# princeton-computational-imaging/Neural-Volume-Super-Resolution

Hardware: AMD Instinct MI355X
Metric: rendered rays/sec (64+128 samples) at 800x800 Lego-like view (higher is better)
Workload: dtype f32 as 2 f16 limbs (3 MFMA products, f32 acc); 1 GPU; Blender-'lego'-like 800x800 view, 64 coarse + 128 fine samples, tri-plane decoder (3x800^2x48 + 32^2x48 planes, 4+4x128 MLP), 1 view per GPU per step; partition=view

## Files before the change

### neural-volume-super-resolution_amd/csrc/render3.hip

```cpp
#include "pair_core.h"

#include "colour_order.h"
#include "occupancy.h"
#include "nvsr_internal.h"

namespace nvsr {

template <int LZ>
__device__ __forceinline__ void render_pass3_body(const SceneDev& sc, const float* __restrict__ packed, long N, int S,
                                                  const float* __restrict__ rays, const float* __restrict__ z, int lindisp,
                                                  const float* __restrict__ noise, int white,
                                                  float* __restrict__ rgb, float* __restrict__ disp,
                                                  float* __restrict__ acc, float* __restrict__ weights,
                                                  float* __restrict__ depth, float* __restrict__ raw_out, unsigned* __restrict__ flag,
                                                  float* __restrict__ live_z = nullptr, float* __restrict__ live_w = nullptr,
                                                  int* __restrict__ live_n = nullptr, const int* __restrict__ group_slot = nullptr,
                                                  const int* __restrict__ pts = nullptr, const int* __restrict__ pt_steps = nullptr, float* views = nullptr,
                                                  const int* __restrict__ kept = nullptr, const int* __restrict__ kept_n = nullptr) {
    constexpr int LIMBS = LZ & 7;
    constexpr bool ZCOMP = (LZ & 8) != 0;
    constexpr int PHASE = (LZ >> 4) & 7;
    constexpr bool FUSED = PHASE == 0, KEPT = PHASE == 4, DENSITY = PHASE == 1 || KEPT, POINTS = PHASE == 3, COLOUR = PHASE == 2 || POINTS;
    constexpr bool F16 = limb_f16(LIMBS);
    using L = Lds3<LIMBS>;
    constexpr int NP = limb_products(LIMBS);
    constexpr int NSF = 3 * 4 * NP, NSH = 4 * 4 * NP;
    __shared__ __attribute__((aligned(16))) unsigned lds[L::TOTAL];
    NVSR_RACE_PROBE_DELAY(lds);
    Ring3<LIMBS> rs{__builtin_amdgcn_make_buffer_rsrc(const_cast<float*>(packed + limb_region(LIMBS)), 0, KB_TOTAL * kb_words(region_limbs(LIMBS)) * 4, 0x00020000),
                    lds, 0, __builtin_amdgcn_readfirstlane((int)(threadIdx.x >> 6)), (int)(threadIdx.x & 63), ring3_voff<LIMBS>(threadIdx.x)};
    float* ldsf = reinterpret_cast<float*>(lds);
    for (int i = threadIdx.x; i < SMALL_FLOATS; i += TPB2) {
        float v = packed[P_SMALL + i] * (!F16 ? 1.0f : i < S_ALPHA_W ? F16_X_SCALE : i < S_HEAD_B ? F16_HEAD_SCALE : 1.0f);
        if (F16 && i >= S_HEAD_B && i < S_HEAD_B + 4) v += packed[P_SMALL + S_F16_POISON];
        ldsf[L::SMALL + i] = v;
    }
    const float* small = ldsf + L::SMALL;

    const int lane0 = rs.lane;
    const unsigned nblk = gridDim.x, xcd = blockIdx.x & 7u, per = nblk >> 3, rem = nblk & 7u;
    unsigned blk_ = xcd * per + (xcd < rem ? xcd : rem) + (blockIdx.x >> 3);
    if constexpr (COLOUR || KEPT) blk_ = (unsigned)__builtin_amdgcn_readfirstlane(group_slot[blockIdx.x]);
    const unsigned blk = blk_;
    const long base = (long)blk * RAYS2 + rs.wave * 64 + (lane0 & 31);
    long rayX = base, rayY = base + 32;
    const bool validX = rayX < N, validY = rayY < N;
    if (!validX) rayX = N - 1;
    if (!validY) rayY = N - 1;
    int nX = 0, nY = 0;
    if constexpr (COLOUR || KEPT) {
        const int* const order = KEPT ? kept_n : live_n;
        const long block_base = (long)(blk / (ORDER_RAYS / RAYS2)) * ORDER_RAYS;
        if (validX) { const int e = order[base]; rayX = block_base + (e & (ORDER_RAYS - 1)); nX = e >> ORDER_SHIFT; }
        if (validY) { const int e = order[base + 32]; rayY = block_base + (e & (ORDER_RAYS - 1)); nY = e >> ORDER_SHIFT; }
    }
    constexpr int RAY3_FLOATS = L::RAY_FLOATS;
    const int ownX = rs.wave * 64 + (lane0 & 31), ownY = ownX + 32;
    float* rcX = ldsf + L::RAYS + ownX * RAY3_FLOATS;
    float* rcY = rcX + 32 * RAY3_FLOATS;
// ... 28 lines not shown
    X.cr = X.cg = X.cb = X.dep = X.ac = 0.0f;
    Y.cr = Y.cg = Y.cb = Y.dep = Y.ac = 0.0f;
    const float* lzX = COLOUR ? live_z + rayX * S : nullptr;
    const float* lzY = COLOUR ? live_z + rayY * S : nullptr;
    const float* lwX = COLOUR ? live_w + rayX * S : nullptr;
    const float* lwY = COLOUR ? live_w + rayY * S : nullptr;
    int trip = S;
    float wX = 0.0f, wY = 0.0f, wXn = 0.0f, wYn = 0.0f;
    auto kept_row = [&](long ray) NVSR_INL -> const int* {
        asm volatile("" : "+v"(ray));
        return kept + ray * S;
    };
    auto z_row = [&](long ray) NVSR_INL -> const float* {
        if constexpr (ZCOMP) return nullptr;
        asm volatile("" : "+v"(ray));
        return z + ray * S;
    };
    int idxX = 0, idxY = 0, idxXn = 0, idxYn = 0, cX = 0, cY = 0;
    bool actX = false, actY = false;
    auto kept_at = [&](const int* kp, int k, int prev) NVSR_INL -> int { const int e = kp[k < S ? k : S - 1]; return e < 0 ? prev : e; };
    auto live_depth = [&](const float* lzp, const float* rc, int n, int k) NVSR_INL -> float {
        if (n == 0) return rc[7];
        const float e = lzp[k < n ? k : n - 1];
        if constexpr (ZCOMP) return depth_of(nullptr, rc, __float_as_int(e));
        else return e;
    };
    auto live_weight = [](const float* lwp, int n, int k) NVSR_INL -> float { return n == 0 ? 0.0f : lwp[k < n ? k : n - 1]; };
    int slotX = ownX, slotY = ownY, slotXn = ownX, slotYn = ownY, eX1 = POINT_NONE, eY1 = POINT_NONE;
    bool liveX = false, liveY = false, liveXn = false, liveYn = false;
    float* const pt_sums = ldsf + L::PTS;
    float* const pt_exch = pt_sums + 3 * RAYS2;
    int* const pt_slot = reinterpret_cast<int*>(pt_exch + 3 * RAYS2);
    int* const pt_ray = pt_slot + RAYS2;
    const long pt_block = (long)(blk / (ORDER_RAYS / RAYS2)) * ORDER_RAYS;
    const int* const peX = POINTS ? pts + (long)blk * RAYS2 * S + ownX : nullptr;
    auto point_of = [&](int e, int own, int& slot, bool& live, float& zv, float& wv) NVSR_INL {
        live = e != POINT_NONE;
        slot = live ? (int)((unsigned)e >> 24) : own;
        const float* rc = ldsf + L::RAYS + slot * RAY3_FLOATS;
        zv = rc[7]; wv = 0.0f;
        if (live) {
            const long at = (pt_block + pt_ray[slot]) * S + (e & 0xffffff);
            const float ze = live_z[at];
            wv = live_w[at];
            if constexpr (ZCOMP) zv = coarse_depth(rc[7], L::FAR >= 0 ? ldsf[L::FAR + slot] : rc[16], __float_as_int(ze), S, lindisp);
            else zv = ze;
        }
    };
    auto load_view = [&](int slot, float (&V)[HALF_C]) NVSR_INL {
        const f32x4* vp = reinterpret_cast<const f32x4*>(views + ((long)blk * RAYS2 + slot) * POINT_VIEW_FLOATS + HALF_C * (lane0 >> 5));
#pragma unroll
        for (int i = 0; i < HALF_C / 4; ++i) { const f32x4 v = vp[i]; V[4 * i] = v[0]; V[4 * i + 1] = v[1]; V[4 * i + 2] = v[2]; V[4 * i + 3] = v[3]; }
    };
    if constexpr (POINTS) {
        static_assert(!R3_BOUNCE, "the points' LDS region is the f16 kernels' bounce slot");
        trip = __builtin_amdgcn_readfirstlane(pt_steps[blk]);
        __syncthreads();
    } else if constexpr (COLOUR || KEPT) {
        __shared__ int trip_s[NW2];
        int m = max(nX, nY);
#pragma unroll
        for (int o = 16; o >= 1; o >>= 1) m = max(m, __shfl_xor(m, o));
        if (lane0 == 0) trip_s[rs.wave] = m;
        __syncthreads();
        trip = __builtin_amdgcn_readfirstlane(max(max(trip_s[0], trip_s[1]), max(trip_s[2], trip_s[3])));
        if constexpr (KEPT) {
            const int* kX = kept_row(rayX);
            const int* kY = kept_row(rayY);
            actX = nX > 0; actY = nY > 0;
            idxX = kept_at(kX, 0, 0); idxY = kept_at(kY, 0, 0);
            idxXn = kept_at(kX, 1, idxX); idxYn = kept_at(kY, 1, idxY);
            X.zc = depth_of(z_row(rayX), rcX, idxX); Y.zc = depth_of(z_row(rayY), rcY, idxY);
        } else {
            X.zc = live_depth(lzX, rcX, nX, 0); Y.zc = live_depth(lzY, rcY, nY, 0);
            wX = live_weight(lwX, nX, 0); wY = live_weight(lwY, nY, 0);
        }
    } else {
        if constexpr (ZCOMP) __syncthreads();
        X.zc = depth_of(zX, rcX, 0); Y.zc = depth_of(zY, rcY, 0);
    }
    RawTaps4 rt;
    RawTaps2 r2;

    auto point_norm = [&](const float* rc, float zc, float& n0, float& n1, float& n2) NVSR_INL {
        const f32x4 c0 = reinterpret_cast<const f32x4*>(rc)[0], c1 = reinterpret_cast<const f32x4*>(rc)[1];
        n0 = norm_coord(__fadd_rn(c0[0], __fmul_rn(c0[3], zc)), sc.lo[0], sc.range[0]);
        n1 = norm_coord(__fadd_rn(c0[1], __fmul_rn(c1[0], zc)), sc.lo[1], sc.range[1]);
        n2 = norm_coord(__fadd_rn(c0[2], __fmul_rn(c1[1], zc)), sc.lo[2], sc.range[2]);
    };
    auto scale_taps = [](Taps& t) NVSR_INL {
        if constexpr (F16) { t.nw *= F16_X_SCALE; t.ne *= F16_X_SCALE; t.sw *= F16_X_SCALE; t.se *= F16_X_SCALE; }
    };
    auto view_job = [&](const float* rtp) NVSR_INL {
        const f32x4 c2 = reinterpret_cast<const f32x4*>(rtp)[0], c3 = reinterpret_cast<const f32x4*>(rtp)[1];
        GatherJob j;
        j.plane = sc.plane[3];
        j.t.o00 = __float_as_int(c2[0]); j.t.o01 = __float_as_int(c2[1]); j.t.o10 = __float_as_int(c2[2]); j.t.o11 = __float_as_int(c2[3]);
        j.t.nw = c3[0]; j.t.ne = c3[1]; j.t.sw = c3[2]; j.t.se = c3[3];
        scale_taps(j.t);
        return j;
    };

    __syncthreads();
    if constexpr (!DENSITY) {
#pragma unroll
        for (int k2 = 0; k2 < 2; ++k2) {
            Tile3& t = k2 ? Y : X;
            const GatherJob vj = view_job(k2 ? rtY : rtX);
// ... 16 lines not shown
                for (int c = 0; c < 3; ++c) pt_sums[ownX * 3 + c] = pt_sums[ownY * 3 + c] = 0.0f;
                pt_ray[ownX] = (int)(rayX - pt_block); pt_ray[ownY] = (int)(rayY - pt_block);
            }
            __syncthreads();
            const int eX0 = trip > 0 ? peX[0] : POINT_NONE, eY0 = trip > 0 ? peX[32] : POINT_NONE;
            eX1 = trip > 1 ? peX[RAYS2] : POINT_NONE; eY1 = trip > 1 ? peX[RAYS2 + 32] : POINT_NONE;
            point_of(eX0, ownX, slotX, liveX, X.zc, wX);
            point_of(eY0, ownY, slotY, liveY, Y.zc, wY);
            load_view(slotX, X.V); load_view(slotY, Y.V);
        }
    } else {
#pragma unroll
        for (int k2 = 0; k2 < 2; ++k2) {
            Tile3& t = k2 ? Y : X;
            float n0, n1, n2;
            point_norm(k2 ? rcY : rcX, t.zc, n0, n1, n2);
#pragma unroll
            for (int p = 0; p < 3; ++p) {
                GatherJob pj;
                pj.plane = sc.plane[p]; pj.t = pos_taps2(sc, p, n0, n1, n2); scale_taps(pj.t);
#pragma unroll
                for (int k = 0; k < 12; ++k) gather4_load(k, pj, lane0 >> 5, rt);
#pragma unroll
                for (int c = 0; c < HALF_C; ++c) gather4_blend(c, pj, rt, t.F);
#pragma unroll
                for (int c = 0; c < HALF_C; ++c) {
                    t.D[c] = p == 0 ? t.F[c] : p == 1 ? __fadd_rn(t.D[c], t.F[c]) : div3(__fadd_rn(t.D[c], t.F[c]));
                    asm volatile("" : "+v"(t.D[c]));
                }
                __builtin_amdgcn_sched_barrier(0);
            }
        }
    }
    auto head_out = [](float v) NVSR_INL { if constexpr (LIMBS == 1) return fabsf(v) == __builtin_inff() ? __builtin_nanf("") : v; else return v; };
    Limbs<LIMBS> cur, fa;
    f32x2_t nsc = {-F16_ACC_UNSCALE, -F16_ACC_UNSCALE};
    asm volatile("" : "+s"(nsc));
#if R3_STAMP
    float stamp[8] = {0, 0, 0, 0, 0, 0, 0, 0};
    unsigned long long tprev = __builtin_amdgcn_s_memtime();
#endif
    constexpr bool RESIDENT = L::RES_KB > 0 && !DENSITY;
    constexpr bool DRES = DENSITY && L::DEN_RES_KB > 0;
    static_assert(!DRES || L::DEN_RES_KB == 9, "the split of layer 1 chunk b below is written for 3 + 4 + 2 resident K-blocks");
    constexpr int KB_FIRST = DRES ? KB_DEN0 + L::DEN_RES_KB : DENSITY ? KB_DEN0 : RESIDENT ? KB_RGB0 + 9 : KB_RGB0;
    constexpr int NKB_FIRST = DRES ? KB_DEN1 + 8 - KB_FIRST : 3;
    unsigned* const res = lds + L::RES;
    if constexpr (RESIDENT) ring3_load_resident<LIMBS, L::RES_KB>(rs, res, KB_RGB0);
    if constexpr (DRES) ring3_load_resident<LIMBS, L::DEN_RES_KB>(rs, res, KB_DEN0);
    unsigned* cw = const_cast<unsigned*>(ring3_issue<LIMBS, NKB_FIRST>(rs, KB_FIRST));
    if constexpr (DRES) ring3_sync<NKB_FIRST * LIMBS>();
    const int steps = COLOUR || KEPT ? trip : S;
    for (int s = 0; s < steps; ++s) {
        asm volatile("" : "+v"(rs.voff), "+v"(rs.lane));
#if R3_NO_VIEW_HOIST
        if constexpr (!POINTS) {
#pragma unroll
        for (int c = 0; c < HALF_C; ++c) asm volatile("" : "+v"(X.V[c]), "+v"(Y.V[c]));
        }
#endif
        if constexpr (POINTS) { rcX = ldsf + L::RAYS + slotX * RAY3_FLOATS; rcY = ldsf + L::RAYS + slotY * RAY3_FLOATS; }
        const int lane = rs.lane, h = lane >> 5;
        const bool last = (s + 1 == S);
        if constexpr (!COLOUR && !KEPT) {
            X.zn = depth_of(zX, rcX, last ? s : s + 1);
            Y.zn = depth_of(zY, rcY, last ? s : s + 1);
        }
        const float nzX = !COLOUR && noise ? noise[rayX * S + s] : 0.0f;
        const float nzY = !COLOUR && noise ? noise[rayY * S + s] : 0.0f;
        float xn0, xn1, xn2, yn0, yn1, yn2;
        if constexpr (!KEPT) {
            point_norm(rcX, DENSITY ? X.zn : X.zc, xn0, xn1, xn2);
            point_norm(rcY, DENSITY ? Y.zn : Y.zc, yn0, yn1, yn2);
        }
        BiasPend4 bp;
        bp.slot = bounce_slot(ldsf + L::VTAPS + rs.wave * 64 * L::TAP_FLOATS + lane * 4);
        HeadPend<3> hp3;
        HeadPend<1> hp1;
        SplitPend tp;

        auto feat = [](const float (&f)[HALF_C]) NVSR_INL { return [&f](int kb, int i) NVSR_INL { return f[8 * kb + i]; }; };
        auto hid = [](const f32x16 (&a)[4], int kb0) NVSR_INL { return [&a, kb0](int kb, int i) NVSR_INL { const int k = kb0 + kb; return a[k >> 1][8 * (k & 1) + i]; }; };
        auto split_feat = [&](const float (&f)[HALF_C]) NVSR_INL { split_all<LIMBS>([&f](int i) NVSR_INL { return f[i]; }, cur); };
        auto tail_of = [&](const f32x16 (&a)[4], int kb) NVSR_INL {
            return [&a, kb, &tp](int slice, Limbs<LIMBS>& nxt) NVSR_INL { split_slice<LIMBS>(slice, [&a, kb](int i) NVSR_INL { return a[kb >> 1][8 * (kb & 1) + i]; }, nxt, tp); };
        };
        auto none = [](int) NVSR_INL {};

        GatherJob ja, jb;
        R3_MARK(0)
        if constexpr (!DRES) ring3_sync<(ZCOMP || COLOUR || KEPT) ? 0 : 2>();
        int eX2 = POINT_NONE, eY2 = POINT_NONE;
        if constexpr (POINTS) {
            if (s + 2 < steps) { eX2 = peX[(s + 2) * RAYS2]; eY2 = peX[(s + 2) * RAYS2 + 32]; }
            point_of(eX1, ownX, slotXn, liveXn, X.zn, wXn);
            point_of(eY1, ownY, slotYn, liveYn, Y.zn, wYn);
        } else if constexpr (COLOUR) {
            X.zn = live_depth(lzX, rcX, nX, s + 1); Y.zn = live_depth(lzY, rcY, nY, s + 1);
            wXn = live_weight(lwX, nX, s + 1); wYn = live_weight(lwY, nY, s + 1);
        } else if constexpr (KEPT) {
            X.zn = depth_of(z_row(rayX), rcX, idxXn); Y.zn = depth_of(z_row(rayY), rcY, idxYn);
            point_norm(rcX, X.zn, xn0, xn1, xn2);
            point_norm(rcY, Y.zn, yn0, yn1, yn2);
        }
        unsigned* nw = (RESIDENT || DENSITY) ? nullptr : ring3_take(rs);
        float hx[3] = {0.0f, 0.0f, 0.0f};
        if constexpr (!DENSITY) {
        const unsigned* const w_view = RESIDENT ? res : cw;
        R3_MARK(1)
        R3_RESET
#define NVSR_ROLL(TL, JL, TB, JB, LOADS, BLENDS) [&](int slot) NVSR_INL { gather_roll<NSF, LOADS, BLENDS, F16 && R3_BLEND_PK>(slot, JL, TL.F, JB, TB.F, h, rt); }
#define NVSR_ROLL_DMA(TL, JL, TB, JB, LOADS, BLENDS, NKB, KB0) \
        [&](int slot) NVSR_INL { gather_roll<NSF, LOADS, BLENDS, F16 && R3_BLEND_PK>(slot, JL, TL.F, JB, TB.F, h, rt); dma_side<LIMBS, NKB>(slot, rs, nw, KB0); }
        ja.plane = sc.plane[0]; ja.t = pos_taps2(sc, 0, xn0, xn1, xn2); scale_taps(ja.t);
        split_feat(X.V);
        if constexpr (RESIDENT) limb_block<LIMBS, 3, true, true>(w_view, lane, X.acc, cur, fa, feat(X.V), NVSR_ROLL(X, ja, Y, jb, true, false), NoTail{});
        else limb_block<LIMBS, 3, true, true>(cw, lane, X.acc, cur, fa, feat(X.V), NVSR_ROLL_DMA(X, ja, Y, jb, true, false, 3, KB_RGB0 + 3), NoTail{});
        R3_MARKB(0)
        if constexpr (POINTS) load_view(slotXn, X.V);
        jb.plane = sc.plane[0]; jb.t = pos_taps2(sc, 0, yn0, yn1, yn2); scale_taps(jb.t);
        split_feat(Y.V);
        limb_block<LIMBS, 3, true, false>(w_view, lane, Y.acc, cur, fa, feat(Y.V), NVSR_ROLL(Y, jb, X, ja, true, true), NoTail{});
        R3_MARKB(1)
        if constexpr (POINTS) load_view(slotYn, Y.V);
        const unsigned* w_p0 = res + 3 * kb_words(LIMBS);
        if constexpr (!RESIDENT) {
            cw = nw;
            ring3_sync<YOUNGER_THAN_CHUNK>();
            nw = ring3_take(rs);
            w_p0 = cw;
        }
#pragma unroll
        for (int c = 0; c < HALF_C; ++c) X.D[c] = X.F[c];
        ja.plane = sc.plane[1]; ja.t = pos_taps2(sc, 1, xn0, xn1, xn2); scale_taps(ja.t);
        split_feat(X.F);
        if constexpr (RESIDENT) limb_block<LIMBS, 3, false, true>(w_p0, lane, X.acc, cur, fa, feat(X.F), NVSR_ROLL(X, ja, Y, jb, true, true), NoTail{});
        else limb_block<LIMBS, 3, false, true>(cw, lane, X.acc, cur, fa, feat(X.F), NVSR_ROLL_DMA(X, ja, Y, jb, true, true, 3, KB_RGB0 + 6), NoTail{});
        R3_MARKB(2)
#pragma unroll
        for (int c = 0; c < HALF_C; ++c) Y.D[c] = Y.F[c];
        jb.plane = sc.plane[1]; jb.t = pos_taps2(sc, 1, yn0, yn1, yn2); scale_taps(jb.t);
        split_feat(Y.F);
        limb_block<LIMBS, 3, false, false>(w_p0, lane, Y.acc, cur, fa, feat(Y.F), NVSR_ROLL(Y, jb, X, ja, true, true), NoTail{});
        R3_MARKB(3)
        const unsigned* w_p1 = res + 6 * kb_words(LIMBS);
        if constexpr (!RESIDENT) {
            cw = nw;
            ring3_sync<YOUNGER_THAN_CHUNK>();
            nw = ring3_take(rs);
            w_p1 = cw;
        }
#pragma unroll
        for (int c = 0; c < HALF_C; ++c) X.D[c] = __fadd_rn(X.D[c], X.F[c]);
        ja.plane = sc.plane[2]; ja.t = pos_taps2(sc, 2, xn0, xn1, xn2); scale_taps(ja.t);
        split_feat(X.F);
        if constexpr (RESIDENT) limb_block<LIMBS, 3, false, true>(w_p1, lane, X.acc, cur, fa, feat(X.F), NVSR_ROLL(X, ja, Y, jb, true, true), NoTail{});
        else limb_block<LIMBS, 3, false, true>(cw, lane, X.acc, cur, fa, feat(X.F), NVSR_ROLL_DMA(X, ja, Y, jb, true, true, 3, KB_RGB0 + 9), NoTail{});
        R3_MARKB(4)
#pragma unroll
        for (int c = 0; c < HALF_C; ++c) Y.D[c] = __fadd_rn(Y.D[c], Y.F[c]);
        jb.plane = sc.plane[2]; jb.t = pos_taps2(sc, 2, yn0, yn1, yn2); scale_taps(jb.t);
        split_feat(Y.F);
        limb_block<LIMBS, 3, false, false>(w_p1, lane, Y.acc, cur, fa, feat(Y.F), NVSR_ROLL(Y, jb, X, ja, true, true), NoTail{});
        R3_MARKB(5)
        if constexpr (!RESIDENT) {
            cw = nw;
            ring3_sync<YOUNGER_THAN_CHUNK>();
        }
        nw = ring3_take(rs);
#pragma unroll
        for (int c = 0; c < HALF_C; ++c) X.D[c] = div3(__fadd_rn(X.D[c], X.F[c]));
        split_feat(X.F);
        limb_block<LIMBS, 3, false, true>(cw, lane, X.acc, cur, fa, feat(X.F), NVSR_ROLL_DMA(X, ja, Y, jb, false, true, 4, KB_RGB1), NoTail{});
        R3_MARKB(6)
#pragma unroll
        for (int c = 0; c < HALF_C; ++c) Y.D[c] = div3(__fadd_rn(Y.D[c], Y.F[c]));
        split_feat(Y.F);
        limb_block<LIMBS, 3, false, false>(cw, lane, Y.acc, cur, fa, feat(Y.F),
                                           [&](int slot) NVSR_INL { spread<RELU_STEPS, 0, NSF>(slot, [&](int k) NVSR_INL { relu_bias_step<LIMBS>(k, small + S_BIAS + 4 * HID, h, X.acc, X.act, bp, nsc); }); },
                                           tail_of(X.act, 0));
        R3_MARKB(7)
        cw = nw;
        R3_MARK(2)
        }

        auto relu_side = [&](Tile3& t, int bias_vec) NVSR_INL {
            return [&, bias_vec](int slot) NVSR_INL { spread<RELU_STEPS, 0, NSH>(slot, [&](int k) NVSR_INL { relu_bias_step<LIMBS>(k, small + S_BIAS + bias_vec * HID, h, t.acc, t.act, bp, nsc); }); };
        };
#define NVSR_HIDDEN_LAYER_(SYNC, XA_SIDE, VPREV, VTHIS, KB_NEXT_A, NKB_A, KB_NEXT_B, NKB_B, X_B_SIDE)                                \
        R3_RESETH                                                                                                                   \
        SYNC;                                                                                                                       \
        R3_MARKH(0)                                                                                                                 \
        nw = ring3_take(rs);                                                                                                        \
        R3_MARKH(1)                                                                                                                 \
        limb_block<LIMBS, 4, true, true>(cw, lane, X.acc, cur, fa, hid(X.act, 0),                                                   \
                                         [&](int slot) NVSR_INL { (XA_SIDE)(slot); dma_side<LIMBS, NKB_A>(slot, rs, nw, KB_NEXT_A); }, tail_of(Y.act, 0)); \
        R3_MARKH(2)                                                                                                                 \
        limb_block<LIMBS, 4, true, false>(cw, lane, Y.acc, cur, fa, hid(Y.act, 0), none, tail_of(X.act, 4));                        \
        R3_MARKH(3)                                                                                                                 \
        cw = nw;                                                                                                                    \
        ring3_sync<0>();                                                                                                               \
        nw = ring3_take(rs);                                                                                                        \
        R3_MARKH(4)                                                                                                                 \
        limb_block<LIMBS, 4, false, true>(cw, lane, X.acc, cur, fa, hid(X.act, 4),                                                  \
                                          [&](int slot) NVSR_INL { dma_side<LIMBS, NKB_B>(slot, rs, nw, KB_NEXT_B); }, tail_of(Y.act, 4));   \
        R3_MARKH(5)                                                                                                                 \
        X_B_SIDE;                                                                                                                   \
        R3_MARKH(6)                                                                                                                 \
        cw = nw;

#define NVSR_HIDDEN_LAYER(VPREV, ...) NVSR_HIDDEN_LAYER_(ring3_sync<0>(), relu_side(Y, VPREV), VPREV, __VA_ARGS__)
#define NVSR_YB_PLAIN(VTHIS) (limb_block<LIMBS, 4, false, false>(cw, lane, Y.acc, cur, fa, hid(Y.act, 4), relu_side(X, VTHIS), tail_of(X.act, 0)))
        if constexpr (!DENSITY) {
        NVSR_HIDDEN_LAYER(4, 5, KB_RGB1 + 4, 4, KB_RGB1 + 8, 4, NVSR_YB_PLAIN(5))
        NVSR_HIDDEN_LAYER(5, 6, KB_RGB1 + 12, 4, KB_RGB1 + 16, 4, NVSR_YB_PLAIN(6))
        NVSR_HIDDEN_LAYER(6, 7, KB_RGB1 + 20, 4, (COLOUR ? KB_FIRST : KB_DEN0), 3,
                          (limb_block<LIMBS, 4, false, false>(cw, lane, Y.acc, cur, fa, hid(Y.act, 4),
                                                              [&](int slot) NVSR_INL {
                                                                  if constexpr (COLOUR) {
                                                                      spread<RELU_STEPS, 0, NSH / 2>(slot, [&](int k) NVSR_INL { relu_bias_step<LIMBS>(k, small + S_BIAS + 7 * HID, h, X.acc, X.act, bp, nsc); });
                                                                      spread<64, NSH / 2, NSH>(slot, [&](int k) NVSR_INL { heads_side<3>(k >> 2, k & 3, small + S_RGB_W, h, X.act, hx, hp3); });
                                                                  } else relu_side(X, 7)(slot);
                                                              },
                                                              NoTail{})))
        }

        R3_MARK(3)
        if constexpr (FUSED) {
        ring3_sync<0>();
        nw = ring3_take(rs);
        split_feat(X.D);
        limb_block<LIMBS, 3, true, true>(cw, lane, X.acc, cur, fa, feat(X.D),
                                         [&](int slot) NVSR_INL {
                                             spread<RELU_STEPS, 0, NSF>(slot, [&](int k) NVSR_INL { relu_bias_step<LIMBS>(k, small + S_BIAS + 7 * HID, h, Y.acc, Y.act, bp, nsc); });
                                             spread<64, 0, NSF>(slot, [&](int k) NVSR_INL { heads_side<3>(k >> 2, k & 3, small + S_RGB_W, h, X.act, hx, hp3); });
                                             dma_side<LIMBS, 4>(slot, rs, nw, KB_DEN1);
                                         },
                                         NoTail{});
#pragma unroll
        for (int c = 0; c < 3; ++c) X.raw[c] = head_out((hx[c] + __shfl_xor(hx[c], 32)) + small[S_HEAD_B + 1 + c]);
        float hy[3] = {0.0f, 0.0f, 0.0f};
        split_feat(Y.D);
        limb_block<LIMBS, 3, true, false>(cw, lane, Y.acc, cur, fa, feat(Y.D),
                                          [&](int slot) NVSR_INL {
                                              spread<64, 0, NSF>(slot, [&](int k) NVSR_INL { heads_side<3>(k >> 2, k & 3, small + S_RGB_W, h, Y.act, hy, hp3); });
                                              spread<RELU_STEPS, 0, NSF>(slot, [&](int k) NVSR_INL { relu_bias_step<LIMBS>(k, small + S_BIAS + 0 * HID, h, X.acc, X.act, bp, nsc); });
                                          },
                                          tail_of(X.act, 0));
#pragma unroll
        for (int c = 0; c < 3; ++c) Y.raw[c] = head_out((hy[c] + __shfl_xor(hy[c], 32)) + small[S_HEAD_B + 1 + c]);
        cw = nw;

        R3_MARK(4)
        NVSR_HIDDEN_LAYER(0, 1, KB_DEN1 + 4, 4, KB_DEN1 + 8, 4, NVSR_YB_PLAIN(1))
        NVSR_HIDDEN_LAYER(1, 2, KB_DEN1 + 12, 4, KB_DEN1 + 16, 4, NVSR_YB_PLAIN(2))
        } else if constexpr (DENSITY) {
        float (&Fg)[HALF_C] = X.F;
#define NVSR_HALF(JL, HL, JB, HB, LOADS, BLENDS, NS_) gather_half<NS_, LOADS, HL, BLENDS, HB>(slot, JL, JB, Fg, h, r2)
#define NVSR_JOB(J, P, N0, N1, N2) J.plane = sc.plane[P]; J.t = pos_taps2(sc, P, N0, N1, N2); scale_taps(J.t);
        const unsigned* const w_d0 = DRES ? res : cw;
        if constexpr (!DRES) nw = ring3_take(rs);
        NVSR_JOB(ja, 0, xn0, xn1, xn2)
        split_feat(X.D);
        limb_block<LIMBS, 3, true, true>(w_d0, lane, X.acc, cur, fa, feat(X.D),
                                         [&](int slot) NVSR_INL {
                                             NVSR_HALF(ja, 0, ja, 0, true, false, NSF);
                                             if constexpr (!DRES) dma_side<LIMBS, 4>(slot, rs, nw, KB_DEN1);
                                         },
                                         NoTail{});
        split_feat(Y.D);
        limb_block<LIMBS, 3, true, false>(w_d0, lane, Y.acc, cur, fa, feat(Y.D),
                                          [&](int slot) NVSR_INL {
                                              spread<RELU_STEPS, 0, NSF>(slot, [&](int k) NVSR_INL { relu_bias_step<LIMBS>(k, small + S_BIAS + 0 * HID, h, X.acc, X.act, bp, nsc); });
                                              NVSR_HALF(ja, 1, ja, 0, true, true, NSF);
                                          },
                                          tail_of(X.act, 0));
        if constexpr (!DRES) cw = nw;
#define NVSR_DEN_LAYER(VPREV, KB_NEXT_A, KB_NEXT_B, NKB_B, PRE_XA, G_XA, PRE_YA, G_YA, PRE_XB, G_XB, PRE_YB, YB_SIDE, YB_TAIL)                      \
        ring3_sync<12>();                                                                                                           \
        nw = ring3_take(rs);                                                                                                        \
        PRE_XA                                                                                                                      \
        limb_block<LIMBS, 4, true, true>(cw, lane, X.acc, cur, fa, hid(X.act, 0),                                                   \
                                         [&](int slot) NVSR_INL { relu_side(Y, VPREV)(slot); G_XA; dma_side<LIMBS, 4>(slot, rs, nw, KB_NEXT_A); }, tail_of(Y.act, 0)); \
        PRE_YA                                                                                                                      \
        limb_block<LIMBS, 4, true, false>(cw, lane, Y.acc, cur, fa, hid(Y.act, 0), [&](int slot) NVSR_INL { G_YA; }, tail_of(X.act, 4)); \
        cw = nw;                                                                                                                    \
        ring3_sync<12>();                                                                                                           \
        nw = ring3_take(rs);                                                                                                        \
        PRE_XB                                                                                                                      \
        limb_block<LIMBS, 4, false, true>(cw, lane, X.acc, cur, fa, hid(X.act, 4),                                                  \
                                          [&](int slot) NVSR_INL { G_XB; dma_side<LIMBS, NKB_B>(slot, rs, nw, KB_NEXT_B); }, tail_of(Y.act, 4)); \
        PRE_YB                                                                                                                      \
        limb_block<LIMBS, 4, false, false>(cw, lane, Y.acc, cur, fa, hid(Y.act, 4), [&](int slot) NVSR_INL { YB_SIDE; }, YB_TAIL);     \
        cw = nw;
#define NVSR_D_SET(T) _Pragma("unroll") for (int c = 0; c < HALF_C; ++c) { T.D[c] = Fg[c]; asm volatile("" : "+v"(T.D[c])); }
#define NVSR_D_ADD(T) _Pragma("unroll") for (int c = 0; c < HALF_C; ++c) { T.D[c] = __fadd_rn(T.D[c], Fg[c]); asm volatile("" : "+v"(T.D[c])); }
#define NVSR_D_AVG(T) _Pragma("unroll") for (int c = 0; c < HALF_C; ++c) { T.D[c] = div3(__fadd_rn(T.D[c], Fg[c])); asm volatile("" : "+v"(T.D[c])); }
        if constexpr (DRES) {
            const unsigned* const w_1a = res + 3 * kb_words(LIMBS);
            const unsigned* const w_1b = res + 7 * kb_words(LIMBS);
            NVSR_JOB(jb, 1, xn0, xn1, xn2)
            limb_block<LIMBS, 4, true, true>(w_1a, lane, X.acc, cur, fa, hid(X.act, 0),
                                             [&](int slot) NVSR_INL { relu_side(Y, 0)(slot); NVSR_HALF(jb, 0, ja, 1, true, true, NSH); }, tail_of(Y.act, 0));
            NVSR_D_SET(X)
            limb_block<LIMBS, 4, true, false>(w_1a, lane, Y.acc, cur, fa, hid(Y.act, 0), [&](int slot) NVSR_INL { NVSR_HALF(jb, 1, jb, 0, true, true, NSH); },
                                              tail_of(X.act, 4));
            NVSR_JOB(ja, 2, xn0, xn1, xn2)
            limb_block<LIMBS, 2, false, true>(w_1b, lane, X.acc, cur, fa, hid(X.act, 4), [&](int slot) NVSR_INL { NVSR_HALF(ja, 0, jb, 1, true, true, NSH); },
// ... 5 lines not shown
                                                  const int slot = sl + NSH / 2;
                                                  NVSR_HALF(ja, 0, jb, 1, true, true, NSH);
                                                  dma_side<LIMBS, 4>(sl, rs, nw, KB_DEN1 + 8);
                                              },
                                              tail_of(Y.act, 4));
            NVSR_D_ADD(X)
            limb_block<LIMBS, 2, false, true>(w_1b, lane, Y.acc, cur, fa, hid(Y.act, 4),
                                              [&](int slot) NVSR_INL { relu_side(X, 1)(slot); NVSR_HALF(ja, 1, ja, 0, true, true, NSH); }, tail_of(Y.act, 6));
            limb_block<LIMBS, 2, false, true>(cw, lane, Y.acc, cur, fa, hid(Y.act, 6),
                                              [&](int sl) NVSR_INL {
                                                  const int slot = sl + NSH / 2;
                                                  relu_side(X, 1)(slot); NVSR_HALF(ja, 1, ja, 0, true, true, NSH);
                                              },
                                              tail_of(X.act, 0));
            cw = nw;
        } else {
        NVSR_DEN_LAYER(0, KB_DEN1 + 4, KB_DEN1 + 8, 4,
                       NVSR_JOB(jb, 1, xn0, xn1, xn2), NVSR_HALF(jb, 0, ja, 1, true, true, NSH),
                       NVSR_D_SET(X), NVSR_HALF(jb, 1, jb, 0, true, true, NSH),
                       NVSR_JOB(ja, 2, xn0, xn1, xn2), NVSR_HALF(ja, 0, jb, 1, true, true, NSH),
                       NVSR_D_ADD(X), relu_side(X, 1)(slot); NVSR_HALF(ja, 1, ja, 0, true, true, NSH), tail_of(X.act, 0))
        }
        NVSR_DEN_LAYER(1, KB_DEN1 + 12, KB_DEN1 + 16, 4,
                       NVSR_JOB(jb, 0, yn0, yn1, yn2), NVSR_HALF(jb, 0, ja, 1, true, true, NSH),
                       NVSR_D_AVG(X), NVSR_HALF(jb, 1, jb, 0, true, true, NSH),
                       NVSR_JOB(ja, 1, yn0, yn1, yn2), NVSR_HALF(ja, 0, jb, 1, true, true, NSH),
                       NVSR_D_SET(Y), relu_side(X, 2)(slot); NVSR_HALF(ja, 1, ja, 0, true, true, NSH), tail_of(X.act, 0))
        float sx[1] = {0.0f};
        auto sigma_side = [&](int slot) NVSR_INL {
            spread<RELU_STEPS, 0, NSH / 2>(slot, [&](int k) NVSR_INL { relu_bias_step<LIMBS>(k, small + S_BIAS + 3 * HID, h, X.acc, X.act, bp, nsc); });
            spread<64, NSH / 2, NSH>(slot, [&](int k) NVSR_INL { heads_side<1>(k >> 2, k & 3, small + S_ALPHA_W, h, X.act, sx, hp1); });
        };
        NVSR_DEN_LAYER(2, KB_DEN1 + 20, KB_FIRST, NKB_FIRST,
                       NVSR_JOB(jb, 2, yn0, yn1, yn2), NVSR_HALF(jb, 0, ja, 1, true, true, NSH),
                       NVSR_D_ADD(Y), NVSR_HALF(jb, 1, jb, 0, true, true, NSH),
                       , NVSR_HALF(jb, 1, jb, 1, false, true, NSH),
                       NVSR_D_AVG(Y), sigma_side(slot), NoTail{})
#undef NVSR_DEN_LAYER
#undef NVSR_D_SET
#undef NVSR_D_ADD
#undef NVSR_D_AVG
#undef NVSR_HALF
#undef NVSR_JOB
        X.raw[3] = head_out((sx[0] + __shfl_xor(sx[0], 32)) + small[S_HEAD_B]);
        }
        if constexpr (FUSED) {
        float sx[1] = {0.0f};
        NVSR_HIDDEN_LAYER(2, 3, KB_DEN1 + 20, 4, KB_FIRST, 3,
                          (limb_block<LIMBS, 4, false, false>(cw, lane, Y.acc, cur, fa, hid(Y.act, 4),
                                                              [&](int slot) NVSR_INL {
                                                                  spread<RELU_STEPS, 0, NSH / 2>(slot, [&](int k) NVSR_INL { relu_bias_step<LIMBS>(k, small + S_BIAS + 3 * HID, h, X.acc, X.act, bp, nsc); });
                                                                  spread<64, NSH / 2, NSH>(slot, [&](int k) NVSR_INL { heads_side<1>(k >> 2, k & 3, small + S_ALPHA_W, h, X.act, sx, hp1); });
                                                              },
                                                              NoTail{})))
        X.raw[3] = head_out((sx[0] + __shfl_xor(sx[0], 32)) + small[S_HEAD_B]);
        }
        R3_MARK(5)
        if constexpr (!COLOUR) {

        float zsX = 0.0f, zsY = 0.0f;
        int e1X = 0, e1Y = 0, e2X = 0, e2Y = 0;
        const bool lastX = KEPT ? idxX + 1 == S : last, lastY = KEPT ? idxY + 1 == S : last;
        if constexpr (KEPT) {
            zsX = depth_of(z_row(rayX), rcX, lastX ? idxX : idxX + 1); zsY = depth_of(z_row(rayY), rcY, lastY ? idxY : idxY + 1);
            { const int* kX = kept_row(rayX); e1X = kX[s + 1 < S ? s + 1 : S - 1]; e2X = kX[s + 2 < S ? s + 2 : S - 1]; }
            { const int* kY = kept_row(rayY); e1Y = kY[s + 1 < S ? s + 1 : S - 1]; e2Y = kY[s + 2 < S ? s + 2 : S - 1]; }
        }
#pragma unroll
        for (int k = 0; k < RELU_STEPS; ++k) relu_bias_step<LIMBS>(k, small + S_BIAS + 3 * HID, h, Y.acc, Y.act, bp, nsc);
        {
            float hd[1];
            head_dots<1>(small + S_ALPHA_W, h, Y.act, hd);
            Y.raw[3] = head_out(hd[0] + small[S_HEAD_B]);
        }
        if (raw_out && lane < 32) {
            if (validX) *reinterpret_cast<f32x4*>(raw_out + (rayX * S + s) * 4) = f32x4{X.raw[0], X.raw[1], X.raw[2], X.raw[3]};
            if (validY) *reinterpret_cast<f32x4*>(raw_out + (rayY * S + s) * 4) = f32x4{Y.raw[0], Y.raw[1], Y.raw[2], Y.raw[3]};
        }
        if constexpr (!KEPT) actX = actY = true;
        if constexpr (KEPT) {
            {
                const float t0 = X.T, d0 = X.dep, a0 = X.ac, g0 = X.zn;
                X.zn = zsX;
                composite_weight(X, reinterpret_cast<const f32x4*>(rcX)[1][2], 0.0f, lastX);
                X.zn = g0; X.T = actX ? X.T : t0; X.dep = actX ? X.dep : d0; X.ac = actX ? X.ac : a0;
            }
            {
                const float t0 = Y.T, d0 = Y.dep, a0 = Y.ac, g0 = Y.zn;
                Y.zn = zsY;
                composite_weight(Y, reinterpret_cast<const f32x4*>(rcY)[1][2], 0.0f, lastY);
                Y.zn = g0; Y.T = actY ? Y.T : t0; Y.dep = actY ? Y.dep : d0; Y.ac = actY ? Y.ac : a0;
            }
        } else if constexpr (DENSITY) {
            composite_weight(X, reinterpret_cast<const f32x4*>(rcX)[1][2], nzX, last);
            composite_weight(Y, reinterpret_cast<const f32x4*>(rcY)[1][2], nzY, last);
        } else {
            composite_sample(X, reinterpret_cast<const f32x4*>(rcX)[1][2], nzX, last);
            composite_sample(Y, reinterpret_cast<const f32x4*>(rcY)[1][2], nzY, last);
        }
        if (weights && lane < 32) {
            if (validX && actX) weights[rayX * S + (KEPT ? idxX : s)] = X.raw[3];
            if (validY && actY) weights[rayY * S + (KEPT ? idxY : s)] = Y.raw[3];
        }
        if constexpr (DENSITY) {
            const bool liveX = actX && !(X.raw[3] == 0.0f), liveY = actY && !(Y.raw[3] == 0.0f);
            if (lane < 32) {
                if (validX && liveX) { live_z[rayX * S + cX] = ZCOMP ? __int_as_float(KEPT ? idxX : s) : X.zc; live_w[rayX * S + cX] = X.raw[3]; }
                if (validY && liveY) { live_z[rayY * S + cY] = ZCOMP ? __int_as_float(KEPT ? idxY : s) : Y.zc; live_w[rayY * S + cY] = Y.raw[3]; }
            }
            cX += liveX; cY += liveY;
            if constexpr (KEPT) {
                actX = validX && s + 1 < S && e1X >= 0; actY = validY && s + 1 < S && e1Y >= 0;
                idxX = e1X < 0 ? idxX : e1X; idxY = e1Y < 0 ? idxY : e1Y;
                idxXn = e2X < 0 ? idxX : e2X; idxYn = e2Y < 0 ? idxY : e2Y;
            }
        }
        } else {
#pragma unroll
        for (int c = 0; c < 3; ++c) X.raw[c] = head_out((hx[c] + __shfl_xor(hx[c], 32)) + small[S_HEAD_B + 1 + c]);
#pragma unroll
        for (int k = 0; k < RELU_STEPS; ++k) relu_bias_step<LIMBS>(k, small + S_BIAS + 7 * HID, h, Y.acc, Y.act, bp, nsc);
        {
            float hd[3];
            head_dots<3>(small + S_RGB_W, h, Y.act, hd);
#pragma unroll
            for (int c = 0; c < 3; ++c) Y.raw[c] = head_out(hd[c] + small[S_HEAD_B + 1 + c]);
        }
        if constexpr (POINTS) {
            if (lane < 32) {
#pragma unroll
                for (int c = 0; c < 3; ++c) { pt_exch[ownX * 3 + c] = colour_term(wX, X.raw[c]); pt_exch[ownY * 3 + c] = colour_term(wY, Y.raw[c]); }
                pt_slot[ownX] = liveX ? slotX : -1; pt_slot[ownY] = liveY ? slotY : -1;
            }
            __syncthreads();
            const int p = rs.wave * 64 + lane, sl = pt_slot[p];
            if (sl >= 0 && (p == 0 || pt_slot[p - 1] != sl)) {
                float a0 = pt_sums[sl * 3], a1 = pt_sums[sl * 3 + 1], a2 = pt_sums[sl * 3 + 2];
                int q = p;
                do {
                    a0 = __fadd_rn(a0, pt_exch[q * 3]); a1 = __fadd_rn(a1, pt_exch[q * 3 + 1]); a2 = __fadd_rn(a2, pt_exch[q * 3 + 2]);
                    ++q;
                } while (q < RAYS2 && pt_slot[q] == sl);
                pt_sums[sl * 3] = a0; pt_sums[sl * 3 + 1] = a1; pt_sums[sl * 3 + 2] = a2;
            }
            __syncthreads();
            slotX = slotXn; slotY = slotYn; liveX = liveXn; liveY = liveYn; eX1 = eX2; eY1 = eY2;
        } else {
            composite_colour(X, wX, s < nX);
            composite_colour(Y, wY, s < nY);
        }
        wX = wXn; wY = wYn;
        }
#undef NVSR_HIDDEN_LAYER
#undef NVSR_HIDDEN_LAYER_
#undef NVSR_ROLL
#undef NVSR_ROLL_DMA
#undef NVSR_YB_PLAIN
        X.zc = X.zn; Y.zc = Y.zn;
        R3_MARK(6)
    }
#if R3_STAMP
    if (raw_out && rs.lane < 32 && validX) {
        for (int i = 0; i < 8; ++i) raw_out[(rayX * S + (i >> 2)) * 4 + (i & 3)] = stamp[i] / (float)S;
    }
#endif
    asm volatile("s_waitcnt vmcnt(0)" ::: "memory");

    if constexpr (POINTS) {
        if (rs.lane < 32) {
            X.cr = pt_sums[ownX * 3]; X.cg = pt_sums[ownX * 3 + 1]; X.cb = pt_sums[ownX * 3 + 2];
            Y.cr = pt_sums[ownY * 3]; Y.cg = pt_sums[ownY * 3 + 1]; Y.cb = pt_sums[ownY * 3 + 2];
        }
    }
    if (rs.lane < 32) {
#pragma unroll
        for (int k = 0; k < 2; ++k) {
            const Tile3& t = k ? Y : X;
            const long ray = k ? rayY : rayX;
            if (!(k ? validY : validX)) continue;
            float cr = t.cr, cg = t.cg, cb = t.cb;
            const float ac = COLOUR ? acc[ray] : t.ac;
            if constexpr (!COLOUR) {
                const float q = t.dep / t.ac;
                disp[ray] = 1.0f / ((q != q) ? q : fmaxf(1e-10f, q));
                acc[ray] = t.ac;
                if (depth) depth[ray] = t.dep;
            }
            if constexpr (DENSITY) {
                live_n[ray] = k ? cY : cX;
                cr = cg = cb = 0.0f;
            } else {
                if (white) { const float bg = 1.0f - ac; cr += bg; cg += bg; cb += bg; }
                rgb[ray * 3 + 0] = cr; rgb[ray * 3 + 1] = cg; rgb[ray * 3 + 2] = cb;
            }
            if (F16 && flag && !(fabsf(cr + cg + cb + ac) <= 3.0e38f)) __hip_atomic_fetch_or(flag, 1u, __ATOMIC_RELAXED, __HIP_MEMORY_SCOPE_AGENT);
        }
    }
}

template <int LIMBS>
__global__ __launch_bounds__(TPB2, 1) void render_pass3_coarse_kernel(SceneDev sc, const float* __restrict__ packed, long N, int S,
                                                                     const float* __restrict__ rays, const float* __restrict__ z,
                                                                     const float* __restrict__ noise, int white,
                                                                     float* __restrict__ rgb, float* __restrict__ disp,
                                                                     float* __restrict__ acc, float* __restrict__ weights,
                                                                     float* __restrict__ depth, float* __restrict__ raw_out, unsigned* __restrict__ flag) {
    render_pass3_body<LIMBS>(sc, packed, N, S, rays, z, 0, noise, white, rgb, disp, acc, weights, depth, raw_out, flag);
}
template <int LIMBS>
__global__ __launch_bounds__(TPB2, 1) void render_pass3_coarse_z_kernel(SceneDev sc, const float* __restrict__ packed, long N, int S,
                                                                       const float* __restrict__ rays, int lindisp,
                                                                       const float* __restrict__ noise, int white,
                                                                       float* __restrict__ rgb, float* __restrict__ disp,
                                                                       float* __restrict__ acc, float* __restrict__ weights,
                                                                       float* __restrict__ depth, float* __restrict__ raw_out, unsigned* __restrict__ flag) {
#if defined(__HIP_DEVICE_COMPILE__)
    render_pass3_body<LIMBS + 8>(sc, packed, N, S, rays, nullptr, lindisp, noise, white, rgb, disp, acc, weights, depth, raw_out, flag);
#endif
}
template <int LIMBS>
__global__ __launch_bounds__(TPB2, 1) void render_pass3_kernel(SceneDev sc, const float* __restrict__ packed, long N, int S,
                                                              const float* __restrict__ rays, const float* __restrict__ z,
                                                              const float* __restrict__ noise, int white,
                                                              float* __restrict__ rgb, float* __restrict__ disp,
                                                              float* __restrict__ acc, float* __restrict__ depth,
                                                              float* __restrict__ raw_out, unsigned* __restrict__ flag) {
    render_pass3_body<LIMBS>(sc, packed, N, S, rays, z, 0, noise, white, rgb, disp, acc, nullptr, depth, raw_out, flag);
}

template <int LIMBS>
__global__ __launch_bounds__(TPB2, 1) void render_pass3_density_kernel(SceneDev sc, const float* __restrict__ packed, long N, int S,
                                                                      const float* __restrict__ rays, const float* __restrict__ z,
                                                                      const float* __restrict__ noise, float* __restrict__ disp,
                                                                      float* __restrict__ acc, float* __restrict__ weights,
                                                                      float* __restrict__ depth, unsigned* __restrict__ flag,
                                                                      float* __restrict__ live_z, float* __restrict__ live_w, int* __restrict__ live_n) {
#if defined(__HIP_DEVICE_COMPILE__)
    render_pass3_body<LIMBS + 16>(sc, packed, N, S, rays, z, 0, noise, 0, nullptr, disp, acc, weights, depth, nullptr, flag, live_z, live_w, live_n);
#endif
}
template <int LIMBS>
__global__ __launch_bounds__(TPB2, 1) void render_pass3_density_z_kernel(SceneDev sc, const float* __restrict__ packed, long N, int S,
                                                                        const float* __restrict__ rays, int lindisp,
                                                                        const float* __restrict__ noise, float* __restrict__ disp,
                                                                        float* __restrict__ acc, float* __restrict__ weights,
                                                                        float* __restrict__ depth, unsigned* __restrict__ flag,
                                                                        float* __restrict__ live_z, float* __restrict__ live_w, int* __restrict__ live_n) {
#if defined(__HIP_DEVICE_COMPILE__)
    render_pass3_body<LIMBS + 8 + 16>(sc, packed, N, S, rays, nullptr, lindisp, noise, 0, nullptr, disp, acc, weights, depth, nullptr, flag, live_z, live_w, live_n);
#endif
// ... 239 lines not shown
```

Baseline: 8.096 million rays/s.

## Defer POINTS-phase colour head and run-sum reduction into next step's layer-1 pipeline

In the POINTS phase, the last layer's ReLU, the Y-tile colour head dot products and the per-slot run-length colour sum are no longer done at the end of each step behind two block-wide barriers. They are now software-pipelined into the following step: the ReLU and head work ride in the side slots of the first-layer MFMA block, the exchange terms are written right after it, and the run-sum is placed after the first hidden layer's X-A block. The in-loop __syncthreads pair is gone, and an epilogue drains the last pending step. This trades extra live registers and a one-step lag for more overlap and fewer barriers. It relies on existing ring syncs to order the LDS exchange writes and reads.

```diff
diff --git a/neural-volume-super-resolution_amd/csrc/render3.hip b/neural-volume-super-resolution_amd/csrc/render3.hip
--- a/neural-volume-super-resolution_amd/csrc/render3.hip
+++ b/neural-volume-super-resolution_amd/csrc/render3.hip
@@ -5,6 +5,17 @@
 #include "nvsr_internal.h"
 
 namespace nvsr {
+
+constexpr int spread_slot(int step, int nsteps, int ns) {
+    for (int j = 0; j < ns; ++j)
+        if (step < (j + 1) * nsteps / ns) return j;
+    return ns;
+}
+constexpr bool heads_follow_relu(int ns, int lag, int span) {
+    for (int g = 0; g < 16; ++g)
+        if (lag + spread_slot(4 * g + 2, 64, span) < spread_slot(4 * g + 7, RELU_STEPS, ns)) return false;
+    return true;
+}
 
 template <int LZ>
 __device__ __forceinline__ void render_pass3_body(const SceneDev& sc, const float* __restrict__ packed, long N, int S,
@@ -139,8 +150,32 @@
 #pragma unroll
         for (int i = 0; i < HALF_C / 4; ++i) { const f32x4 v = vp[i]; V[4 * i] = v[0]; V[4 * i + 1] = v[1]; V[4 * i + 2] = v[2]; V[4 * i + 3] = v[3]; }
     };
+    float wXp = 0.0f, wYp = 0.0f, hxp[3] = {0.0f, 0.0f, 0.0f};
+    int slXp = -1, slYp = -1;
+    auto put_terms = [&](const float (&rx)[3], const float (&ry)[3]) NVSR_INL {
+        const bool up = rs.lane >= 32;
+        const float w = up ? wYp : wXp;
+        const int own = up ? ownY : ownX;
+#pragma unroll
+        for (int c = 0; c < 3; ++c) pt_exch[own * 3 + c] = colour_term(w, up ? ry[c] : rx[c]);
+        pt_slot[own] = up ? slYp : slXp;
+    };
+    auto run_sums = [&]() NVSR_INL {
+        const int p = rs.wave * 64 + rs.lane, sl = pt_slot[p];
+        if (sl >= 0 && (p == 0 || pt_slot[p - 1] != sl)) {
+            float a0 = pt_sums[sl * 3], a1 = pt_sums[sl * 3 + 1], a2 = pt_sums[sl * 3 + 2];
+            int q = p;
+            do {
+                a0 = __fadd_rn(a0, pt_exch[q * 3]); a1 = __fadd_rn(a1, pt_exch[q * 3 + 1]); a2 = __fadd_rn(a2, pt_exch[q * 3 + 2]);
+                ++q;
+            } while (q < RAYS2 && pt_slot[q] == sl);
+            pt_sums[sl * 3] = a0; pt_sums[sl * 3 + 1] = a1; pt_sums[sl * 3 + 2] = a2;
+        }
+    };
     if constexpr (POINTS) {
         static_assert(!R3_BOUNCE, "the points' LDS region is the f16 kernels' bounce slot");
+#pragma unroll
+        for (int ob = 0; ob < 4; ++ob) Y.acc[ob] = f32x16{0, 0, 0, 0, 0, 0, 0, 0, 0, 0, 0, 0, 0, 0, 0, 0};
         trip = __builtin_amdgcn_readfirstlane(pt_steps[blk]);
         __syncthreads();
     } else if constexpr (COLOUR || KEPT) {
@@ -263,6 +298,9 @@
     if constexpr (DRES) ring3_sync<NKB_FIRST * LIMBS>();
     const int steps = COLOUR || KEPT ? trip : S;
     for (int s = 0; s < steps; ++s) {
+#if R3_STAMP
+        if (s == 0) tprev = __builtin_amdgcn_s_memtime();
+#endif
         asm volatile("" : "+v"(rs.voff), "+v"(rs.lane));
 #if R3_NO_VIEW_HOIST
         if constexpr (!POINTS) {
@@ -323,11 +361,32 @@
 #define NVSR_ROLL(TL, JL, TB, JB, LOADS, BLENDS) [&](int slot) NVSR_INL { gather_roll<NSF, LOADS, BLENDS, F16 && R3_BLEND_PK>(slot, JL, TL.F, JB, TB.F, h, rt); }
 #define NVSR_ROLL_DMA(TL, JL, TB, JB, LOADS, BLENDS, NKB, KB0) \
         [&](int slot) NVSR_INL { gather_roll<NSF, LOADS, BLENDS, F16 && R3_BLEND_PK>(slot, JL, TL.F, JB, TB.F, h, rt); dma_side<LIMBS, NKB>(slot, rs, nw, KB0); }
+#define NVSR_ROLL2(TL, JL, TB, JB, LOADS, BLENDS, MORE) [&](int slot) NVSR_INL { gather_roll<NSF, LOADS, BLENDS, F16 && R3_BLEND_PK>(slot, JL, TL.F, JB, TB.F, h, rt); MORE; }
+#define NVSR_ROLL_DMA2(TL, JL, TB, JB, LOADS, BLENDS, NKB, KB0, MORE) \
+        [&](int slot) NVSR_INL { gather_roll<NSF, LOADS, BLENDS, F16 && R3_BLEND_PK>(slot, JL, TL.F, JB, TB.F, h, rt); dma_side<LIMBS, NKB>(slot, rs, nw, KB0); MORE; }
+        float hy[3] = {0.0f, 0.0f, 0.0f};
+        constexpr int HEAD_LAG = NSF / 6, HEAD_SPAN = NSF - HEAD_LAG;
+        static_assert(heads_follow_relu(NSF, HEAD_LAG, HEAD_SPAN), "a head group would read activations not yet written");
+        auto defer_relu = [&](int slot) NVSR_INL {
+            if constexpr (POINTS) spread<RELU_STEPS, 0, NSF>(slot, [&](int k) NVSR_INL { relu_bias_step<LIMBS>(k, small + S_BIAS + 7 * HID, h, Y.acc, Y.act, bp, nsc); });
+        };
+        auto defer_heads = [&](int slot) NVSR_INL {
+            if constexpr (POINTS) spread<64, HEAD_LAG, HEAD_LAG + HEAD_SPAN>(slot, [&](int k) NVSR_INL { heads_side<3>(k >> 2, k & 3, small + S_RGB_W, h, Y.act, hy, hp3); });
+        };
         ja.plane = sc.plane[0]; ja.t = pos_taps2(sc, 0, xn0, xn1, xn2); scale_taps(ja.t);
         split_feat(X.V);
-        if constexpr (RESIDENT) limb_block<LIMBS, 3, true, true>(w_view, lane, X.acc, cur, fa, feat(X.V), NVSR_ROLL(X, ja, Y, jb, true, false), NoTail{});
-        else limb_block<LIMBS, 3, true, true>(cw, lane, X.acc, cur, fa, feat(X.V), NVSR_ROLL_DMA(X, ja, Y, jb, true, false, 3, KB_RGB0 + 3), NoTail{});
+        if constexpr (RESIDENT) limb_block<LIMBS, 3, true, true>(w_view, lane, X.acc, cur, fa, feat(X.V), NVSR_ROLL2(X, ja, Y, jb, true, false, defer_relu(slot); defer_heads(slot)), NoTail{});
+        else limb_block<LIMBS, 3, true, true>(cw, lane, X.acc, cur, fa, feat(X.V), NVSR_ROLL_DMA2(X, ja, Y, jb, true, false, 3, KB_RGB0 + 3, defer_relu(slot); defer_heads(slot)), NoTail{});
         R3_MARKB(0)
+        if constexpr (POINTS) {
+            float rx[3], ry[3];
+#pragma unroll
+            for (int c = 0; c < 3; ++c) {
+                rx[c] = head_out((hxp[c] + __shfl_xor(hxp[c], 32)) + small[S_HEAD_B + 1 + c]);
+                ry[c] = head_out((hy[c] + __shfl_xor(hy[c], 32)) + small[S_HEAD_B + 1 + c]);
+            }
+            put_terms(rx, ry);
+        }
         if constexpr (POINTS) load_view(slotXn, X.V);
         jb.plane = sc.plane[0]; jb.t = pos_taps2(sc, 0, yn0, yn1, yn2); scale_taps(jb.t);
         split_feat(Y.V);
@@ -398,7 +457,7 @@
         auto relu_side = [&](Tile3& t, int bias_vec) NVSR_INL {
             return [&, bias_vec](int slot) NVSR_INL { spread<RELU_STEPS, 0, NSH>(slot, [&](int k) NVSR_INL { relu_bias_step<LIMBS>(k, small + S_BIAS + bias_vec * HID, h, t.acc, t.act, bp, nsc); }); };
         };
-#define NVSR_HIDDEN_LAYER_(SYNC, XA_SIDE, VPREV, VTHIS, KB_NEXT_A, NKB_A, KB_NEXT_B, NKB_B, X_B_SIDE)                                \
+#define NVSR_HIDDEN_LAYER_(SYNC, XA_SIDE, VPREV, VTHIS, KB_NEXT_A, NKB_A, KB_NEXT_B, NKB_B, X_B_SIDE, AFTER_XA)                      \
         R3_RESETH                                                                                                                   \
         SYNC;                                                                                                                       \
         R3_MARKH(0)                                                                                                                 \
@@ -407,6 +466,7 @@
         limb_block<LIMBS, 4, true, true>(cw, lane, X.acc, cur, fa, hid(X.act, 0),                                                   \
                                          [&](int slot) NVSR_INL { (XA_SIDE)(slot); dma_side<LIMBS, NKB_A>(slot, rs, nw, KB_NEXT_A); }, tail_of(Y.act, 0)); \
         R3_MARKH(2)                                                                                                                 \
+        AFTER_XA                                                                                                                    \
         limb_block<LIMBS, 4, true, false>(cw, lane, Y.acc, cur, fa, hid(Y.act, 0), none, tail_of(X.act, 4));                        \
         R3_MARKH(3)                                                                                                                 \
         cw = nw;                                                                                                                    \
@@ -423,8 +483,8 @@
 #define NVSR_HIDDEN_LAYER(VPREV, ...) NVSR_HIDDEN_LAYER_(ring3_sync<0>(), relu_side(Y, VPREV), VPREV, __VA_ARGS__)
 #define NVSR_YB_PLAIN(VTHIS) (limb_block<LIMBS, 4, false, false>(cw, lane, Y.acc, cur, fa, hid(Y.act, 4), relu_side(X, VTHIS), tail_of(X.act, 0)))
         if constexpr (!DENSITY) {
-        NVSR_HIDDEN_LAYER(4, 5, KB_RGB1 + 4, 4, KB_RGB1 + 8, 4, NVSR_YB_PLAIN(5))
-        NVSR_HIDDEN_LAYER(5, 6, KB_RGB1 + 12, 4, KB_RGB1 + 16, 4, NVSR_YB_PLAIN(6))
+        NVSR_HIDDEN_LAYER(4, 5, KB_RGB1 + 4, 4, KB_RGB1 + 8, 4, NVSR_YB_PLAIN(5), if constexpr (POINTS) run_sums();)
+        NVSR_HIDDEN_LAYER(5, 6, KB_RGB1 + 12, 4, KB_RGB1 + 16, 4, NVSR_YB_PLAIN(6), )
         NVSR_HIDDEN_LAYER(6, 7, KB_RGB1 + 20, 4, (COLOUR ? KB_FIRST : KB_DEN0), 3,
                           (limb_block<LIMBS, 4, false, false>(cw, lane, Y.acc, cur, fa, hid(Y.act, 4),
                                                               [&](int slot) NVSR_INL {
@@ -433,7 +493,7 @@
                                                                       spread<64, NSH / 2, NSH>(slot, [&](int k) NVSR_INL { heads_side<3>(k >> 2, k & 3, small + S_RGB_W, h, X.act, hx, hp3); });
                                                                   } else relu_side(X, 7)(slot);
                                                               },
-                                                              NoTail{})))
+                                                              NoTail{})), )
         }
 
         R3_MARK(3)
@@ -463,8 +523,8 @@
         cw = nw;
 
         R3_MARK(4)
-        NVSR_HIDDEN_LAYER(0, 1, KB_DEN1 + 4, 4, KB_DEN1 + 8, 4, NVSR_YB_PLAIN(1))
-        NVSR_HIDDEN_LAYER(1, 2, KB_DEN1 + 12, 4, KB_DEN1 + 16, 4, NVSR_YB_PLAIN(2))
+        NVSR_HIDDEN_LAYER(0, 1, KB_DEN1 + 4, 4, KB_DEN1 + 8, 4, NVSR_YB_PLAIN(1), )
+        NVSR_HIDDEN_LAYER(1, 2, KB_DEN1 + 12, 4, KB_DEN1 + 16, 4, NVSR_YB_PLAIN(2), )
         } else if constexpr (DENSITY) {
         float (&Fg)[HALF_C] = X.F;
 #define NVSR_HALF(JL, HL, JB, HB, LOADS, BLENDS, NS_) gather_half<NS_, LOADS, HL, BLENDS, HB>(slot, JL, JB, Fg, h, r2)
@@ -576,7 +636,7 @@
                                                                   spread<RELU_STEPS, 0, NSH / 2>(slot, [&](int k) NVSR_INL { relu_bias_step<LIMBS>(k, small + S_BIAS + 3 * HID, h, X.acc, X.act, bp, nsc); });
                                                                   spread<64, NSH / 2, NSH>(slot, [&](int k) NVSR_INL { heads_side<1>(k >> 2, k & 3, small + S_ALPHA_W, h, X.act, sx, hp1); });
                                                               },
-                                                              NoTail{})))
+                                                              NoTail{})), )
         X.raw[3] = head_out((sx[0] + __shfl_xor(sx[0], 32)) + small[S_HEAD_B]);
         }
         R3_MARK(5)
@@ -639,6 +699,13 @@
                 idxXn = e2X < 0 ? idxX : e2X; idxYn = e2Y < 0 ? idxY : e2Y;
             }
         }
+        } else if constexpr (POINTS) {
+#pragma unroll
+        for (int c = 0; c < 3; ++c) hxp[c] = hx[c];
+        wXp = wX; wYp = wY;
+        slXp = liveX ? slotX : -1; slYp = liveY ? slotY : -1;
+        slotX = slotXn; slotY = slotYn; liveX = liveXn; liveY = liveYn; eX1 = eX2; eY1 = eY2;
+        wX = wXn; wY = wYn;
         } else {
 #pragma unroll
         for (int c = 0; c < 3; ++c) X.raw[c] = head_out((hx[c] + __shfl_xor(hx[c], 32)) + small[S_HEAD_B + 1 + c]);
@@ -650,35 +717,16 @@
 #pragma unroll
             for (int c = 0; c < 3; ++c) Y.raw[c] = head_out(hd[c] + small[S_HEAD_B + 1 + c]);
         }
-        if constexpr (POINTS) {
-            if (lane < 32) {
-#pragma unroll
-                for (int c = 0; c < 3; ++c) { pt_exch[ownX * 3 + c] = colour_term(wX, X.raw[c]); pt_exch[ownY * 3 + c] = colour_term(wY, Y.raw[c]); }
-                pt_slot[ownX] = liveX ? slotX : -1; pt_slot[ownY] = liveY ? slotY : -1;
-            }
-            __syncthreads();
-            const int p = rs.wave * 64 + lane, sl = pt_slot[p];
-            if (sl >= 0 && (p == 0 || pt_slot[p - 1] != sl)) {
-                float a0 = pt_sums[sl * 3], a1 = pt_sums[sl * 3 + 1], a2 = pt_sums[sl * 3 + 2];
-                int q = p;
-                do {
-                    a0 = __fadd_rn(a0, pt_exch[q * 3]); a1 = __fadd_rn(a1, pt_exch[q * 3 + 1]); a2 = __fadd_rn(a2, pt_exch[q * 3 + 2]);
-                    ++q;
-                } while (q < RAYS2 && pt_slot[q] == sl);
-                pt_sums[sl * 3] = a0; pt_sums[sl * 3 + 1] = a1; pt_sums[sl * 3 + 2] = a2;
-            }
-            __syncthreads();
-            slotX = slotXn; slotY = slotYn; liveX = liveXn; liveY = liveYn; eX1 = eX2; eY1 = eY2;
-        } else {
-            composite_colour(X, wX, s < nX);
-            composite_colour(Y, wY, s < nY);
-        }
+        composite_colour(X, wX, s < nX);
+        composite_colour(Y, wY, s < nY);
         wX = wXn; wY = wYn;
         }
 #undef NVSR_HIDDEN_LAYER
 #undef NVSR_HIDDEN_LAYER_
 #undef NVSR_ROLL
 #undef NVSR_ROLL_DMA
+#undef NVSR_ROLL2
+#undef NVSR_ROLL_DMA2
 #undef NVSR_YB_PLAIN
         X.zc = X.zn; Y.zc = Y.zn;
         R3_MARK(6)
@@ -691,6 +739,24 @@
     asm volatile("s_waitcnt vmcnt(0)" ::: "memory");
 
     if constexpr (POINTS) {
+        if (steps > 0) {
+            BiasPend4 bp;
+            bp.slot = bounce_slot(ldsf + L::VTAPS + rs.wave * 64 * L::TAP_FLOATS + rs.lane * 4);
+            const int h = rs.lane >> 5;
+#pragma unroll
+            for (int k = 0; k < RELU_STEPS; ++k) relu_bias_step<LIMBS>(k, small + S_BIAS + 7 * HID, h, Y.acc, Y.act, bp, nsc);
+            float hd[3], rx[3], ry[3];
+            head_dots<3>(small + S_RGB_W, h, Y.act, hd);
+#pragma unroll
+            for (int c = 0; c < 3; ++c) {
+                rx[c] = head_out((hxp[c] + __shfl_xor(hxp[c], 32)) + small[S_HEAD_B + 1 + c]);
+                ry[c] = head_out(hd[c] + small[S_HEAD_B + 1 + c]);
+            }
+            put_terms(rx, ry);
+            __syncthreads();
+            run_sums();
+            __syncthreads();
+        }
         if (rs.lane < 32) {
             X.cr = pt_sums[ownX * 3]; X.cg = pt_sums[ownX * 3 + 1]; X.cb = pt_sums[ownX * 3 + 2];
             Y.cr = pt_sums[ownY * 3]; Y.cg = pt_sums[ownY * 3 + 1]; Y.cb = pt_sums[ownY * 3 + 2];
@@ -720,6 +786,19 @@
             if (F16 && flag && !(fabsf(cr + cg + cb + ac) <= 3.0e38f)) __hip_atomic_fetch_or(flag, 1u, __ATOMIC_RELAXED, __HIP_MEMORY_SCOPE_AGENT);
         }
     }
+#if R3_STAMP
+    if constexpr (PHASE == 1 || POINTS) {
+        float tot = 0.0f;
+        for (int i = 0; i < 7; ++i) tot += stamp[i];
+        const float n = steps > 0 ? (float)steps : 1.0f, tail = (stamp[6] + stamp[0]) / n;
+        for (int k = 0; k < 2; ++k) {
+            const long ray = k ? rayY : rayX;
+            if (rs.lane >= 32 || !(k ? validY : validX)) continue;
+            if constexpr (POINTS) { rgb[ray * 3] = tail; rgb[ray * 3 + 1] = tot / n; rgb[ray * 3 + 2] = (float)steps; }
+            else { disp[ray] = tail; acc[ray] = tot / n; }
+        }
+    }
+#endif
 }
 
 template <int LIMBS>
```

After: 8.142 million rays/s (median of 6 runs). About the same (+0.6%).
